# meiqua/pose_refine

Hardware: AMD Instinct MI355X
Metric: refined poses/sec (640x480, 20 ICP iters) (higher is better)
Workload: dtype f32; 1 GPU; obj_06.ply, 256-pose batch per GPU, 640x480 synthetic depth, projective association, 20 ICP iterations (21 passes), solve on device, 2 pose groups; poses_per_gpu=256, global_batch=256, parallelism=pose-shard x1, no data-path collective, no gather (1 rank)

## Files before the change

pose_refine_amd/csrc/icp_pass.hip:

```cpp
#include "pr_launch.h"
#include "icp_accumulate.h"
#include "icp_solve_device.h"

namespace prk {

template <class Scene, bool kNN, int kStack = 0, bool kRobust = false>
__global__ __launch_bounds__(256, PR_PASS_WAVES) void icp_pass_kernel(IcpBatch b, Scene scene)
{
    extern __shared__ __attribute__((aligned(16))) unsigned char lds_raw[];
    __shared__ float wsum[4][kAccStride];

    const uint32_t pose = blockIdx.y;
    const PoseMeta &pm = b.meta[pose];
    const int32_t st = pm.state;
    if (st == kSkip) return;
    const uint32_t n = pm.count;
    const uint32_t ppb = b.steps * kPointsPerStep;
    if ((uint64_t)blockIdx.x * ppb >= n) return;

    const int4 *lds_topo = nullptr;
    int *stk_node = nullptr; float *stk_lb = nullptr;
    if constexpr (kNN && kStack == 0) {
        int4 *dst = reinterpret_cast<int4 *>(lds_raw);
        for (uint32_t i = threadIdx.x; i < scene.lds_nodes; i += kBlockThreads) dst[i] = scene.topo[i];
// ... 44 lines not shown
    const float *p = partial + (size_t)pose * nblk * kAccStride + comp;
    for (uint32_t g0 = 0; g0 < used; g0 += 16) {
        float v[16];
#pragma unroll
        for (uint32_t k = 0; k < 16; ++k) v[k] = (g0 + k < used) ? p[(size_t)(g0 + k) * kAccStride] : 0.0f;
#pragma unroll
        for (uint32_t k = 0; k < 16; ++k) if (g0 + k < used) total += v[k];
    }
    return total;
}

constexpr uint32_t kLoopLanes = 1024, kLoopWaves = kLoopLanes / 64, kLoopHeader = 64;
static_assert(sizeof(DevIcpState) == 20 * sizeof(uint32_t), "the LDS header holds DevIcpState as 20 words");
size_t icp_loop_cu_lds_bytes(uint32_t nblk) { return ((size_t)nblk * 4 * kAccStride + kLoopHeader) * sizeof(float); }
uint32_t icp_loop_cu_lds_blocks(uint32_t nblk, uint32_t steps, int cap)
{
    const size_t fixed = icp_loop_cu_lds_bytes(nblk), block = (size_t)steps * kPointsPerStep * sizeof(pr_vec3);
    if (fixed > kLoopCuLdsBudget || block == 0) return 0;
    const size_t fit = (kLoopCuLdsTotal - fixed) / block;
    uint32_t r = (uint32_t)(fit < nblk ? fit : nblk);
    if (cap >= 0 && (uint32_t)cap < r) r = (uint32_t)cap;
    return r;
}

template <class Scene>
__global__ __launch_bounds__(kLoopLanes) PR_LOOP_CU_ATTR void icp_loop_cu_kernel(IcpBatch b, Scene scene)
{
    extern __shared__ __attribute__((aligned(16))) float loop_lds[];
    const uint32_t pose = blockIdx.x;
    const PoseMeta &pm = b.meta[pose];
    const int32_t st0 = pm.state;
    const uint32_t n = pm.count;
    if (st0 == kSkip || n == 0) return;
    const uint32_t ppb = b.steps * kPointsPerStep;
    const uint32_t items = ((n + ppb - 1) / ppb) * 4u;
    const uint32_t lane = threadIdx.x & 63u;
    const uint32_t wave = __builtin_amdgcn_readfirstlane(threadIdx.x >> 6);
    float *hdr = loop_lds + (size_t)b.nblk * 4 * kAccStride;
    uint32_t *hdw = reinterpret_cast<uint32_t *>(hdr);
    float *cl = reinterpret_cast<float *>(b.cloud + pm.start);
    float *lcl = hdr + kLoopHeader;
    const uint32_t lds_items = b.lds_blocks * 4u;
    bool xf = (st0 == kRunWithTransform) && !b.pre_transformed;
    float M[12];
#pragma unroll
    for (int i = 0; i < 12; ++i) M[i] = xf ? pm.xform[i] : 0.0f;
    if (wave == 0 && lane < 20) hdw[16 + lane] = reinterpret_cast<const uint32_t *>(b.st + pose)[lane];

    const uint32_t last_it = (uint32_t)b.crit.max_iteration;
    uint32_t it = 0;
    for (;; ++it) {
        const bool score_only = it == last_it;
        for (uint32_t item = wave; item < items; item += kLoopWaves) {
            const uint32_t vb = item >> 2, tib = ((item & 3u) << 6) | lane;
            float acc[29];
            float *row = loop_lds + (size_t)item * kAccStride;
            const bool in_lds = item < lds_items;
            if (score_only) {
                if (!in_lds) vb_accumulate_at<Scene, false, 0, true>(tib, acc, cl, cl, n, vb * ppb, b.steps, xf, M, scene, nullptr, nullptr, nullptr, nullptr, xf);
                else if (it == 0) vb_accumulate_at<Scene, false, 0, true, false, true>(tib, acc, cl, lcl, n, vb * ppb, b.steps, xf, M, scene, nullptr, nullptr, nullptr, nullptr, xf);
                else vb_accumulate_at<Scene, false, 0, true>(tib, acc, lcl, lcl, n, vb * ppb, b.steps, xf, M, scene, nullptr, nullptr, nullptr, nullptr, xf);
                wave_reduce<true>(acc, lane, row);
            } else {
                if (!in_lds) vb_accumulate_at<Scene, false, 0>(tib, acc, cl, cl, n, vb * ppb, b.steps, xf, M, scene, nullptr, nullptr, nullptr, nullptr, xf);
                else if (it == 0) vb_accumulate_at<Scene, false, 0, false, false, true>(tib, acc, cl, lcl, n, vb * ppb, b.steps, xf, M, scene, nullptr, nullptr, nullptr, nullptr, xf);
                else vb_accumulate_at<Scene, false, 0>(tib, acc, lcl, lcl, n, vb * ppb, b.steps, xf, M, scene, nullptr, nullptr, nullptr, nullptr, xf);
                wave_reduce(acc, lane, row);
            }
        }
        __syncthreads();
        if (wave == 0) {
            float total = 0.0f;
            if (lane < 29) {
                const float *r = loop_lds + lane;
                for (uint32_t i = 0; i < items; i += 4u, r += 4 * kAccStride)
                    total += ((r[0] + r[kAccStride]) + r[2 * kAccStride]) + r[3 * kAccStride];
            }
            DevIcpState s;
#pragma unroll
            for (int i = 0; i < 16; ++i) s.T[i] = hdr[16 + i];
            s.fitness = hdr[32]; s.rmse = hdr[33]; s.done = (int32_t)hdw[34]; s.passes = (int32_t)hdw[35];
            float E[16];
            const bool finished = pose_iteration_wave(total, n, s, b.crit, it, E);
            if (lane == 0) {
#pragma unroll
                for (int i = 0; i < 16; ++i) hdr[16 + i] = s.T[i];
                hdr[32] = s.fitness; hdr[33] = s.rmse; hdw[35] = (uint32_t)s.passes;
                if (!finished) {
#pragma unroll
                    for (int i = 0; i < 12; ++i) hdr[i] = E[i];
                }
                hdw[12] = (finished || it >= last_it) ? 1u : 0u;
            }
        }
        __syncthreads();
        if (__builtin_amdgcn_readfirstlane(hdw[12]) != 0u) break;
#pragma unroll
        for (int i = 0; i < 12; ++i) M[i] = __int_as_float(__builtin_amdgcn_readfirstlane(__float_as_int(hdr[i])));
        xf = true;
    }
    if (threadIdx.x == 0) {
        DevIcpState s;
#pragma unroll
        for (int i = 0; i < 16; ++i) s.T[i] = hdr[16 + i];
        s.fitness = hdr[32]; s.rmse = hdr[33]; s.done = 1; s.passes = (int32_t)hdw[35];
        b.st[pose] = s;
        PoseMeta *wm = const_cast<PoseMeta *>(b.meta) + pose;
        if (it > 0) {
#pragma unroll
            for (int i = 0; i < 12; ++i) wm->xform[i] = hdr[i];
        }
        wm->state = kSkip;
    }
}
hipError_t launch_icp_loop_cu_proj_packed(const IcpBatch &b, const SceneProjPacked &sc, uint32_t n_poses, hipStream_t s, uint32_t *lds_blocks_used)
{
    if (lds_blocks_used) *lds_blocks_used = 0;
    if (n_poses == 0 || b.nblk == 0) return hipSuccess;
    size_t lds = icp_loop_cu_lds_bytes(b.nblk);
    if (lds > kLoopCuLdsBudget || b.robust_kind != PR_ROBUST_NONE) return hipErrorInvalidValue;
    IcpBatch bb = b;
    const uint32_t most = icp_loop_cu_lds_blocks(b.nblk, b.steps, -1);
    if (bb.lds_blocks > most) bb.lds_blocks = most;
    const size_t image = (size_t)bb.lds_blocks * b.steps * kPointsPerStep * sizeof(pr_vec3);
    const auto fn = icp_loop_cu_kernel<SceneProjPacked>;
    if (lds + image > kLoopCuLdsBudget && !lds_opt_in(reinterpret_cast<const void *>(fn), 0, (uint32_t)kLoopCuLdsTotal)) bb.lds_blocks = 0;
    if (bb.lds_blocks) lds += image;
    if (lds_blocks_used) *lds_blocks_used = bb.lds_blocks;
    hipLaunchKernelGGL(HIP_KERNEL_NAME(icp_loop_cu_kernel<SceneProjPacked>), dim3(n_poses), dim3(kLoopLanes), lds, s, bb, sc);
    return hipGetLastError();
}

__global__ __launch_bounds__(64) void icp_finalize_kernel(const float *__restrict__ partial, const PoseMeta *__restrict__ meta,
                                                          uint32_t nblk, uint32_t ppb, float *__restrict__ sums)
{
    const uint32_t pose = blockIdx.x;
    if (meta[pose].state == kSkip) return;
    const uint32_t n = meta[pose].count;
    const uint32_t used = (n + ppb - 1) / ppb;
    if (threadIdx.x < kAccStride)
        sums[(size_t)pose * kAccStride + threadIdx.x] = (threadIdx.x < 29) ? sum_partials(partial, pose, nblk, used, threadIdx.x) : 0.0f;
}

__global__ __launch_bounds__(64) void icp_finalize_solve_kernel(const float *__restrict__ partial, PoseMeta *__restrict__ meta,
                                                                uint32_t nblk, uint32_t ppb, DevIcpState *__restrict__ st,
                                                                pr_criteria crit, uint32_t iter)
{
    const uint32_t pose = blockIdx.x;
    if (meta[pose].state == kSkip) return;
    const uint32_t n = meta[pose].count;
    const uint32_t used = (n + ppb - 1) / ppb;
    DevIcpState s = st[pose];
    float total = 0.0f;
// ... 163 lines not shown
```

pose_refine_amd/csrc/pr_context.cpp:

```cpp
#include "pr_runtime.h"

namespace prh {
thread_local std::string g_err;
void set_error(const char *fmt, ...)
{
    char buf[512];
    va_list ap; va_start(ap, fmt); vsnprintf(buf, sizeof buf, fmt, ap); va_end(ap);
    g_err = buf;
}
}

namespace prr {

static std::mutex &g_reg_mu_trace() { static std::mutex m; return m; }

namespace {
struct TraceRec { uint64_t ns; const char *tag; uint32_t tid; };
constexpr size_t kTraceCap = 1u << 18;
TraceRec *g_trace = nullptr;
std::atomic<uint64_t> g_trace_n{ 0 };
std::atomic<int> g_trace_state{ 0 };
std::string g_trace_path;
void trace_dump()
{
// ... 10 lines not shown
    if (st == 1) return;
    if (st == 0) {
        std::lock_guard<std::mutex> lk(g_reg_mu_trace());
        st = g_trace_state.load();
        if (st == 0) {
            const char *p = std::getenv("PR_TRACE");
            if (p && *p) { g_trace_path = p; g_trace = new TraceRec[kTraceCap]; std::atexit(trace_dump); st = 2; } else st = 1;
            g_trace_state.store(st, std::memory_order_release);
        }
        if (st == 1) return;
    }
    timespec ts; clock_gettime(CLOCK_MONOTONIC, &ts);
    static thread_local uint32_t tid = (uint32_t)std::hash<std::thread::id>()(std::this_thread::get_id());
    const uint64_t i = g_trace_n.fetch_add(1);
    if (i < kTraceCap) g_trace[i] = TraceRec{ (uint64_t)ts.tv_sec * 1000000000ull + (uint64_t)ts.tv_nsec, tag, tid };
}

WriteLog g_writes;
std::atomic<uint64_t> g_flag_overtook{ 0 };
std::atomic<uint64_t> g_tight_batches{ 0 };
std::atomic<uint64_t> g_band_batches{ 0 };
std::atomic<uint64_t> g_resident_batches{ 0 };
std::atomic<uint32_t> g_loop_lds_blocks{ 0 };
std::atomic<uint32_t> g_nn_lds_nodes{ 0 }, g_nn_stack_depth{ 0 };
std::atomic<uint64_t> g_nn_pass_launches{ 0 };
Options opt;
std::mutex g_reg_mu;
std::vector<Ctx *> g_shared;
int g_default_device = -1;
thread_local Ctx *g = nullptr;
thread_local PrivateCtx tl_private;
std::mutex g_private_mu;
std::vector<Ctx *> g_private;

void ctx_teardown(Ctx *c)
{
    if (!c->ready) return;
    (void)hipSetDevice(c->device);
    hipStreamSynchronize(c->stream);
    for (Slot &sl : c->slots) slot_release(sl);
    for (DevBuf *b : { &c->aabb, &c->aabb_keys, &c->bbox, &c->poses, &c->depth, &c->row_count, &c->row_off, &c->counts, &c->cloud, &c->meta, &c->partial,
                       &c->sums, &c->packed.rec, &c->nn_prev, &c->dstate, &c->dresults, &c->arrive, &c->conv16, &c->conv8, &c->kd_scratch, &c->kd_tmp, &c->nn_full, &c->gather_tmp, &c->nn_counters, &c->scores, &c->multi, &c->ov_bits, &c->ov_box, &c->ov_mat, &c->cov_state, &c->cov_claimed, &c->mesh_sorted, &c->mesh_verts, &c->contours, &c->normals, &c->cmp_keys, &c->cmp_box, &c->cmp_rec, &c->edge_bits, &c->edge_rows, &c->lvl_rows, &c->lvl_counts, &c->lvl_carry, &c->pd_mats, &c->pd_part, &c->pd_rec, &c->ppf_tmp, &c->ppf_out, &c->plane_tmp, &c->seg_tmp, &c->dfilt_tmp, &c->cloud_tmp, &c->vsd_rec, &c->solid_far, &c->solid_rec, &c->info_meta, &c->info_part }) b->release();
    for (NNDerived &d : c->nn_sets) d.release();
    for (PinBuf *b : { &c->h_sums, &c->h_meta, &c->h_counts, &c->h_results, &c->h_dstate, &c->h_poses, &c->h_flags, &c->h_scores, &c->h_multi, &c->h_ov, &c->h_cov, &c->h_contours, &c->h_normals, &c->h_lvl_carry, &c->h_cmp, &c->h_pd_mats, &c->h_pd_rec, &c->h_ppf, &c->h_plane, &c->h_seg, &c->h_dfilt, &c->h_vsd, &c->h_solid, &c->h_info_meta, &c->h_info_out }) b->release();
    c->packed = PackedCache();
    for (auto &gr : c->graphs) destroy_graph(gr);
// ... 189 lines not shown
    if (n == "solve") { if (value != PR_SOLVE_HOST && value != PR_SOLVE_DEVICE) { set_error("solve must be 0 or 1"); return PR_ERR_INVALID; } opt.solve_mode = value; }
    else if (n == "host_worker") opt.host_worker = value ? 1 : 0;
    else if (n == "start_overlap") opt.start_overlap = value;
    else if (n == "points_per_block") { if (value < 1024 || value % 1024) { set_error("points_per_block must be a multiple of 1024"); return PR_ERR_INVALID; } opt.steps = value / 1024; }
    else if (n == "profile") { if (value < 0 || value > 3) { set_error("profile must be 0, 1 (every launch, synchronous calls), 2 (every launch of one call in sample_period) or 3 (every launch, asynchronous batches stay asynchronous)"); return PR_ERR_INVALID; } opt.profile = value; }
    else if (n == "sample_period") opt.sample_period = std::max(1, value);
    else if (n == "scene_cache") opt.scene_cache = value ? 1 : 0;
    else if (n == "nn_lds_nodes") opt.nn_lds_nodes = std::max(0, value);
    else if (n == "nn_lds_records") opt.nn_lds_records = std::max(0, value);
    else if (n == "nn_compact") opt.nn_compact = value ? 1 : 0;
    else if (n == "nn_wide") opt.nn_wide = value ? 1 : 0;
    else if (n == "blocking_wait") opt.blocking_wait = value ? 1 : 0;
    else if (n == "nn_seed") opt.nn_seed = value ? 1 : 0;
    else if (n == "nn_stack") opt.nn_stack = value ? 1 : 0;
    else if (n == "nn_split") opt.nn_split = value ? 1 : 0;
    else if (n == "nn_run") opt.nn_run = std::min(8, std::max(1, value));
    else if (n == "nn_grid") opt.nn_grid = value ? 1 : 0;
    else if (n == "nn_count") opt.nn_count = value ? 1 : 0;
    else if (n == "host_poll") opt.host_poll = value ? 1 : 0;
    else if (n == "graph") opt.use_graph = value ? 1 : 0;
    else if (n == "fused_solve") opt.fused_solve = value ? 1 : 0;
    else if (n == "resident_loop") opt.resident_loop = value ? 1 : 0;
    else if (n == "loop_lds_blocks") opt.loop_lds_blocks = std::max(-1, value);
    else if (n == "sub_batch") opt.sub_batch = std::min(32768, std::max(32, value));
    else if (n == "overlap_pass") opt.overlap_pass = std::max(-1, value);
    else if (n == "pose_groups") opt.pose_groups = std::min(4, std::max(0, value));
    else if (n == "eager_streams") opt.eager_streams = value ? 1 : 0;
    else if (n == "mesh_order") opt.mesh_order = value ? 1 : 0;
    else if (n == "tight_box") opt.tight_box = value ? 1 : 0;
    else if (n == "box_bands") opt.box_bands = value ? 1 : 0;
    else if (n == "ppf_walk") opt.ppf_walk = value ? 1 : 0;
    else if (n == "raster_mode") { if (value < 0 || value > 1) { set_error("raster_mode must be 0 or 1"); return PR_ERR_INVALID; } opt.raster_mode = value; }
    else { set_error("unknown option %s", name); return PR_ERR_INVALID; }
    return PR_OK;
}

int pr_get_option(const char *name, int *value)
{
    std::lock_guard<std::mutex> lk(g_reg_mu);
    if (!name || !value) { set_error("pr_get_option: null argument"); return PR_ERR_INVALID; }
    const std::string n(name);
    if (n == "solve") *value = opt.solve_mode;
    else if (n == "host_worker") *value = opt.host_worker;
    else if (n == "start_overlap") *value = opt.start_overlap;
    else if (n == "points_per_block") *value = opt.steps * 1024;
    else if (n == "profile") *value = opt.profile;
// ... 7 lines not shown
    else if (n == "nn_seed") *value = opt.nn_seed;
    else if (n == "nn_stack") *value = opt.nn_stack;
    else if (n == "nn_split") *value = opt.nn_split;
    else if (n == "nn_run") *value = opt.nn_run;
    else if (n == "nn_grid") *value = opt.nn_grid;
    else if (n == "nn_count") *value = opt.nn_count;
    else if (n == "host_poll") *value = opt.host_poll;
    else if (n == "stat_flag_overtook") *value = (int)std::min<uint64_t>(g_flag_overtook.load(), 0x7fffffffull);
    else if (n == "stat_tight_batches") *value = (int)std::min<uint64_t>(g_tight_batches.load(), 0x7fffffffull);
    else if (n == "box_pack") *value = (int)prk::kBoxPack;
    else if (n == "pose_dist_chunk") *value = (int)prk::kPoseDistChunk;
    else if (n == "raster_mode") *value = opt.raster_mode;
    else if (n == "mesh_order") *value = opt.mesh_order;
    else if (n == "tight_box") *value = opt.tight_box;
    else if (n == "box_bands") *value = opt.box_bands;
    else if (n == "ppf_walk") *value = opt.ppf_walk;
    else if (n == "stat_band_batches") *value = (int)std::min<uint64_t>(g_band_batches.load(), 0x7fffffffull);
    else if (n == "eager_streams") *value = opt.eager_streams;
    else if (n == "graph") *value = opt.use_graph;
    else if (n == "fused_solve") *value = opt.fused_solve;
    else if (n == "resident_loop") *value = opt.resident_loop;
    else if (n == "loop_lds_blocks") *value = opt.loop_lds_blocks;
    else if (n == "stat_loop_lds_blocks") *value = (int)g_loop_lds_blocks.load();
    else if (n == "stat_nn_lds_nodes") *value = (int)g_nn_lds_nodes.load();
    else if (n == "stat_nn_stack_depth") *value = (int)g_nn_stack_depth.load();
    else if (n == "stat_nn_pass_launches") *value = (int)(g_nn_pass_launches.load() & 0x7fffffffull);
    else if (n == "stat_resident_batches") *value = (int)std::min<uint64_t>(g_resident_batches.load(), 0x7fffffffull);
    else if (n == "sub_batch") *value = opt.sub_batch;
    else if (n == "overlap_pass") *value = opt.overlap_pass;
    else if (n == "pose_groups") *value = opt.pose_groups;
    else { set_error("unknown option %s", name); return PR_ERR_INVALID; }
    return PR_OK;
}

int pr_profile_reset(void)
{
    PR_TRY(bind_default());
    std::lock_guard<std::mutex> lk(g->mu);
    g->icp_ms = g->render_ms = g->cloud_ms = 0; g->icp_launches = g->icp_points = g->icp_bytes = 0; g->sample_clock = 0;
    g->gather_ms = 0; g->gather_n = 0; g->gather_ev_used = 0;
    g->icp_launch_us.clear();
    for (double &v : g->nn_part_ms) v = 0;
    g->nn_part_n = 0;
    return PR_OK;
}

// ... 43 lines not shown
```

pose_refine_amd/csrc/pr_internal.h:

```cpp
#pragma once

#include <hip/hip_runtime_api.h>
#include <hip/hip_vector_types.h>
#include <stddef.h>
#include <stdint.h>
#include <vector>

#include "pose_refine.h"
#include "pr_tuning.h"

namespace prk {

constexpr uint32_t kBlockThreads   = 256;
constexpr uint32_t kPointsPerLane  = 4;
constexpr uint32_t kPointsPerStep  = kBlockThreads * kPointsPerLane;
constexpr uint32_t kAccStride      = 32;
constexpr uint32_t kCloudAlign     = 32;
constexpr uint32_t kBoxPack        = 32;
constexpr uint32_t kQCountStride   = 4;
constexpr uint32_t kNNWordsPerPoint = 6;

enum : int32_t { kSkip = 0, kRun = 1, kRunWithTransform = 2 };

struct alignas(64) PoseMeta {
// ... 26 lines not shown
    float          *nn_slack;
    uint2          *nn_queue;
    uint32_t       *nn_qcount;
    uint2          *nn_queue2;
    uint32_t        pre_transformed;
    pr_criteria     crit;
    uint32_t        robust_kind;
    float           robust_c, robust_inv_c;
    uint32_t        lds_blocks;
};
struct RobustArgs { uint32_t kind; float c, inv_c; float *corr; };

struct SceneProjAoS {
    uint32_t width, height;
    float max_dist_diff, fx, fy, cx, cy;
    float tlx, tly;
    const pr_vec3 *pcd, *normal;
};
struct SceneProjPacked {
    uint32_t width, height;
    float max_dist_diff, fx, fy, cx, cy;
    float tlx, tly;
    const float4 *rec;
    const float *colf, *rowf;
};
struct SceneNNDev {
    float max_dist_diff;
    const int4   *topo;
    const float4 *bmin, *bmax;
    const float4 *pts;
    const pr_vec3 *pcd, *normal;
    uint32_t n_nodes;
    uint32_t lds_nodes;
    const float4 *rec;
    uint32_t stack_depth;
    const uint4 *rec32;
    float qmin[3], qscale[3];
    const uint2 *desc;
    const float4 *grid;
    uint32_t gw, gh;
    float gfx, gfy, gcx, gcy;
    const float4 *pyr4, *pyr16, *pyr64;
    const uint4 *wide;
    uint32_t n_wide;
    float wmin[3], wscale;
    unsigned long long *counters;
// ... 139 lines not shown
hipError_t launch_stage_words(const void *src_host_mapped, void *dst, size_t bytes, hipStream_t s);
hipError_t launch_stage_words64(const void *src_host_mapped, void *dst, size_t bytes, hipStream_t s);
hipError_t launch_copy_words32(const void *src, void *dst, uint32_t n_words, hipStream_t s);
hipError_t launch_d2c_pack_starts(const uint32_t *counts, uint32_t n, PoseMeta *meta, hipStream_t s);
hipError_t launch_emit_box(const int32_t *depth, uint32_t n_poses, uint32_t width, uint32_t height, const int4 *bbox, float fx, float fy,
                           float cx, float cy, const uint32_t *row_count, const uint32_t *row_off, pr_vec3 *cloud, const PoseMeta *meta,
                           hipStream_t s, const uint32_t *box_off = nullptr, bool bands = false);

struct PyramidStrides { uint32_t n; uint32_t s[PR_PYRAMID_MAX_LEVELS]; };
struct alignas(64) PyramidCarry { float T[12]; uint32_t start; uint32_t pad[3]; };
static_assert(sizeof(PyramidCarry) == 64, "PyramidCarry must stay one 64-byte record");
hipError_t launch_pyramid_counts(const int32_t *depth, const int4 *bbox, const uint32_t *box_off, uint32_t n_poses, uint32_t width, uint32_t height,
                                 const PyramidStrides &lv, uint32_t *row_count, uint32_t *row_off, uint32_t *counts, hipStream_t s);
hipError_t launch_pyramid_emit(const int32_t *depth, uint32_t n_poses, uint32_t width, uint32_t height, const int4 *bbox, const uint32_t *box_off,
                               float fx, float fy, float cx, float cy, uint32_t stride, const uint32_t *row_count, const uint32_t *row_off,
                               const PyramidCarry *carry, bool apply, pr_vec3 *cloud, hipStream_t s);

hipError_t launch_icp_pass_proj_aos(const IcpBatch &b, const SceneProjAoS &sc, uint32_t n_poses, hipStream_t s);
hipError_t launch_icp_pass_proj_packed(const IcpBatch &b, const SceneProjPacked &sc, uint32_t n_poses, hipStream_t s);
constexpr size_t kLoopCuLdsBudget = 64u << 10;
size_t icp_loop_cu_lds_bytes(uint32_t nblk);
constexpr size_t kLoopCuLdsTotal = 160u << 10;
uint32_t icp_loop_cu_lds_blocks(uint32_t nblk, uint32_t steps, int cap);
hipError_t launch_icp_loop_cu_proj_packed(const IcpBatch &b, const SceneProjPacked &sc, uint32_t n_poses, hipStream_t s, uint32_t *lds_blocks_used = nullptr);
constexpr uint32_t kPassStaticLds = 4 * kAccStride * (uint32_t)sizeof(float);
constexpr uint32_t kNNLdsNodesMax = 8192;
constexpr uint32_t kNNLdsNodesPlain = ((64u << 10) - kPassStaticLds) / 16u;
struct NNPassRan { uint32_t lds_nodes, stack_depth; };
hipError_t launch_icp_pass_nn(const IcpBatch &b, const SceneNNDev &sc, uint32_t n_poses, hipStream_t s, NNPassRan *ran = nullptr);
hipError_t launch_nn_search(const IcpBatch &b, const SceneNNDev &sc, uint32_t n_poses, uint32_t max_points, uint32_t run, hipStream_t s, hipEvent_t *marks = nullptr);
hipError_t launch_icp_pass_nn_winners(const IcpBatch &b, const SceneNNWinners &sc, uint32_t n_poses, hipStream_t s);
hipError_t launch_icp_pass_grid(const IcpBatch &b, const SceneGridDev &sc, uint32_t n_poses, hipStream_t s);
hipError_t launch_grid_build(const SceneNNDev &tree, float reach, const SceneGridDev &grid, uint32_t *cell_point, hipStream_t s);
hipError_t launch_grid_records(const pr_vec3 *pcd, const pr_vec3 *normal, uint32_t n, float4 *rec, hipStream_t s);
hipError_t launch_contrib29_grid(pr_vec3 *cloud, uint32_t n, const float *update12, const SceneGridDev &sc, float *out, hipStream_t s);
hipError_t launch_contrib29_proj_aos(pr_vec3 *cloud, uint32_t n, const float *update12, const SceneProjAoS &sc, float *out, hipStream_t s);
hipError_t launch_contrib29_proj_packed(pr_vec3 *cloud, uint32_t n, const float *update12, const SceneProjPacked &sc, float *out, hipStream_t s);
hipError_t launch_contrib29_nn(pr_vec3 *cloud, uint32_t n, const float *update12, const SceneNNDev &sc, float *out, hipStream_t s);
hipError_t launch_robust_terms_proj_aos(pr_vec3 *cloud, uint32_t n, const float *update12, const SceneProjAoS &sc, const RobustArgs &ra, float *out, hipStream_t s);
hipError_t launch_robust_terms_proj_packed(pr_vec3 *cloud, uint32_t n, const float *update12, const SceneProjPacked &sc, const RobustArgs &ra, float *out, hipStream_t s);
hipError_t launch_robust_terms_nn(pr_vec3 *cloud, uint32_t n, const float *update12, const SceneNNDev &sc, const RobustArgs &ra, float *out, hipStream_t s);
hipError_t launch_robust_terms_grid(pr_vec3 *cloud, uint32_t n, const float *update12, const SceneGridDev &sc, const RobustArgs &ra, float *out, hipStream_t s);
hipError_t launch_pose_iteration_debug(const float *sums, const uint32_t *n_points, uint32_t n, pr_criteria crit, uint32_t iter, pr_result *state,
                                       float *update, uint32_t *finished, hipStream_t s);
size_t nn_grid_cells(uint32_t gw, uint32_t gh);
hipError_t launch_build_nn_grid(const pr_vec3 *pcd, uint32_t n_points, uint32_t gw, uint32_t gh, float fx, float fy, float cx, float cy,
                                int32_t *cell_idx, float4 *grid, uint32_t *usable, hipStream_t s);
// ... 84 lines not shown
```

pose_refine_amd/csrc/pr_refine.cpp:

```cpp
#include "pr_runtime.h"
#include "pose_box.h"

namespace prr {

int stage_poses(const pr_mat4 *poses_host, size_t n)
{
    PR_TRY(g->poses.ensure(sizeof(pr_mat4) * n));
    PR_TRY(g->h_poses.ensure(sizeof(pr_mat4) * n));
    std::memcpy(g->h_poses.p, poses_host, sizeof(pr_mat4) * n);
    HIP_TRY(prk::launch_stage_words(g->h_poses.dev, g->poses.p, sizeof(pr_mat4) * n, g->stream));
    return PR_OK;
}

uint32_t depth_chunk(size_t img, uint32_t P)
{
    return (uint32_t)std::max<size_t>(1, std::min<size_t>(P, ((size_t)4 << 30) / (img * sizeof(int32_t))));
}

std::pair<size_t, size_t> image_extent(pr_roi roi, size_t W, size_t H)
{
    if (roi.width > 0 && roi.height > 0) return { (size_t)roi.width, (size_t)roi.height };
    return { W, H };
}

// ... 910 lines not shown
    const prk::BoxRows rows{ sl.row_count.as<uint32_t>(), sl.row_off.as<uint32_t>(), sl.counts.as<uint32_t>() + q0, meta, dstate, arrive };
    HIP_TRY(prk::launch_render_boxes(mesh, d_poses + q0, nq, d_box + q0, target, rows, st, false, q0 == 0 ? &chk : nullptr));
    if (timed) { sl.spans.end(te, kSpanRender, q0, nq, false, st); te = sl.spans.begin(st); }
    HIP_TRY(prk::launch_emit_box(sl.depth.as<int32_t>(), nq, W, H, d_box + q0, K[0], K[4], K[2], K[5], sl.row_count.as<uint32_t>(),
                                 sl.row_off.as<uint32_t>(), sl.cloud.as<pr_vec3>(), meta, st, d_off + q0, bands));
    if (timed) sl.spans.end(te, kSpanCloud, q0, nq, false, st);
    if (timed && q0 == 0)
        for (Slot &o : g->slots) if (&o != &sl && o.pending && !o.delivered && o.done) HIP_TRY(hipStreamWaitEvent(st, o.done, 0));

    const uint32_t n_groups = pose_group_count(job.scene_kind, nq, timed);
    if (nn_prev) HIP_TRY(prk::launch_fill_i32(reinterpret_cast<int32_t *>(nn_prev + nl.qcount), (size_t)prk::kQCountStride * nq, 0, st));
    prk::IcpBatch b{};
    b.cloud = sl.cloud.as<pr_vec3>(); b.partial = sl.partial.as<float>(); b.nblk = pl.nblk; b.grid_x = pl.grid_x; b.steps = pl.steps;
    if (nn_prev) nn_carve(b, nn_prev, nl);
    const uint32_t last_pass = (uint32_t)job.crit.max_iteration;
    if (opt.resident_loop && opt.fused_solve && !timed && job.scene_kind == PR_SCENE_PROJ && sc.kind == PR_SCENE_PROJ && sc.packed
        && prk::icp_loop_cu_lds_bytes(pl.nblk) <= prk::kLoopCuLdsBudget) {
        b.meta = meta; b.st = dstate; b.crit = job.crit; b.fused = 1;
        const bool release = q0 + pl.sub >= P;
#if PR_RESIDENT_RELEASE_AHEAD
        if (release) { HIP_TRY(hipEventRecord(sl.progress, st)); sl.progress_valid = true; }
#endif
        b.lds_blocks = prk::icp_loop_cu_lds_blocks(pl.nblk, pl.steps, opt.loop_lds_blocks);
        uint32_t lds_blocks_used = 0;
        HIP_TRY(prk::launch_icp_loop_cu_proj_packed(b, sc.pk, nq, st, &lds_blocks_used));
        g_loop_lds_blocks.store(lds_blocks_used);
#if !PR_RESIDENT_RELEASE_AHEAD
        if (release) { HIP_TRY(hipEventRecord(sl.progress, st)); sl.progress_valid = true; }
#endif
        g_resident_batches.fetch_add(1);
        return PR_OK;
    }
    auto pass = [&](const prk::IcpBatch &bb, uint32_t p0, uint32_t np, hipStream_t gs) -> int {
        if (!timed) { HIP_TRY(launch_pass(bb, sc, np, gs)); return PR_OK; }
        const size_t e0 = sl.spans.begin(st);
        size_t mi[3] = { 0, 0, 0 }; hipEvent_t me[3] = { nullptr, nullptr, nullptr };
        const bool marks = sc.kind == PR_SCENE_NN && sc.nn_split && bb.nn_prev && np <= 32768u && sl.spans.reserve_marks(mi, me);
        HIP_TRY(launch_pass(bb, sc, np, gs, marks ? me : nullptr));
        sl.spans.end(e0, kSpanIcp, q0 + p0, np, bb.iter == 0 || bb.iter == last_pass, st, marks ? mi : nullptr);
        return PR_OK;
    };
    const uint32_t release_pass = release_pass_for(job.mesh.n_tris, nq, g->cloud_hint, job.crit, job.scene_kind, timed, pipeline_start, opt.start_overlap, opt.overlap_pass);
    auto after = [&](uint32_t it, bool &) -> int {
        if (q0 + pl.sub >= P && it == release_pass) { HIP_TRY(hipEventRecord(sl.progress, st)); sl.progress_valid = true; }
        return PR_OK;
    };
    const Lanes lanes{ sl.stream, sl.side, sl.fork, sl.join };
    return device_solve_loop(lanes, n_groups, b, nq, job.crit, opt.fused_solve != 0, meta, dstate, arrive, pass, after);
}
// ... 594 lines not shown
        if (rc == PR_OK) rc = make_job("pr_refine_submit", tris_dev, n_tris, width, height, proj, K, scene_kind, scene, crit, roi, results_dev, job);
        if (rc == PR_OK) rc = refine_submit(g->slots[slot], job, poses_host, n_poses, results_host, cloud_sizes_host);
    }
    trace_mark("pr_refine_submit: exit");
    return rc;
}

int pr_refine_submit(int slot, const pr_triangle *tris_dev, size_t n_tris, const pr_mat4 *poses_host, uint32_t n_poses, uint32_t width, uint32_t height,
                     const pr_mat4 *proj, const float K[9], int scene_kind, const void *scene, pr_criteria crit,
                     pr_result *results_host, pr_result *results_dev, uint32_t *cloud_sizes_host)
{
    return pr_refine_submit_roi(slot, tris_dev, n_tris, poses_host, n_poses, width, height, proj, K, scene_kind, scene, crit, pr_roi{ 0, 0, 0, 0 }, results_host, results_dev, cloud_sizes_host);
}

int pr_refine_wait(int slot)
{
    trace_mark("pr_refine_wait: enter");
    int rc;
    { PR_ENTER(); rc = refine_wait(slot); }
    trace_mark("pr_refine_wait: exit");
    return rc;
}

}
```

pose_refine_amd/csrc/pr_runtime.h:

```cpp
#pragma once
#include <hip/hip_runtime_api.h>
#include <rccl/rccl.h>
#include <dlfcn.h>

#include <algorithm>
#include <atomic>
#include <cfloat>
#include <cmath>
#include <cstdarg>
#include <cstdio>
#include <cstdlib>
#include <cstring>
#include <condition_variable>
#include <memory>
#include <mutex>
#include <thread>
#include <string>
#include <vector>

#include "pr_internal.h"
#include "pr_tuning.h"
#include "pose_box.h"
#include "contour_fit.h"

// ... 66 lines not shown
        if (bytes == 0) {
            void *base = nullptr; size_t size = 0;
            if (hipMemGetAddressRange(reinterpret_cast<hipDeviceptr_t *>(&base), &size, const_cast<void *>(p)) == hipSuccess && base) { lo = reinterpret_cast<uintptr_t>(base); hi = lo + size; }
            else { (void)hipGetLastError(); lo = 0; hi = ~(uintptr_t)0; }
        }
        std::lock_guard<std::mutex> lk(mu);
        ++gen;
        ring[gen % kRing] = W{ lo, hi };
    }
    uint64_t now() { std::lock_guard<std::mutex> lk(mu); return gen; }
    bool written_since(uint64_t since, const void *p, size_t bytes)
    {
        const uintptr_t lo = reinterpret_cast<uintptr_t>(p), hi = lo + bytes;
        std::lock_guard<std::mutex> lk(mu);
        if (gen - since >= kRing) return true;
        for (uint64_t k = since + 1; k <= gen; ++k) { const W &w = ring[k % kRing]; if (w.lo < hi && lo < w.hi) return true; }
        return false;
    }
};
extern WriteLog g_writes;
extern std::atomic<uint64_t> g_tight_batches;
extern std::atomic<uint64_t> g_band_batches;
extern std::atomic<uint64_t> g_resident_batches;
extern std::atomic<uint32_t> g_loop_lds_blocks;
extern std::atomic<uint32_t> g_nn_lds_nodes, g_nn_stack_depth;
extern std::atomic<uint64_t> g_nn_pass_launches;
extern std::atomic<uint64_t> g_flag_overtook;

constexpr int kSlots = PR_SLOTS;
struct Options {
    int pose_groups = 0;
    int solve_mode = PR_SOLVE_HOST;
    int host_worker = 1;
    int steps = 3;
    int profile = 0;
    int sample_period = 32;
    int nn_lds_nodes = 1024;
    int nn_lds_records = 0;
    int nn_seed = 1;
    int nn_compact = 1;
    int blocking_wait = 0;
    int nn_wide = 1;
    int nn_stack = 1;
    int nn_split = 1;
    int nn_run = 8;
    int nn_grid = 1;
    int host_poll = 1;
    int nn_count = 0;
    int start_overlap = -1;
    int overlap_pass = -1;
    int sub_batch = 512;
    int fused_solve = 1;
    int resident_loop = 1;
    int loop_lds_blocks = -1;
    int use_graph = 1;
    int eager_streams = 1;
    int raster_mode = 0;
    int mesh_order = 1;
    int tight_box = 1;
    int box_bands = 1;
    int ppf_walk = 1;
    int scene_cache = 1;
};
extern Options opt;
inline uint32_t pose_groups_for(int scene_kind) { (void)scene_kind; return opt.pose_groups > 0 ? (uint32_t)opt.pose_groups : 2u; }

struct ProjTail { uint32_t exact; prk::FpWords fp; uint32_t pad[3]; };
static_assert(sizeof(ProjTail) == 32, "ProjTail: the 32 bytes behind the tables");
struct PackedLayout { size_t colf, rowf, tail, bytes; };
inline PackedLayout packed_layout(size_t w, size_t h)
{
    PackedLayout l{};
    l.colf = w * h * sizeof(float4); l.rowf = l.colf + w * sizeof(float);
    l.tail = l.colf + (((w + h) * sizeof(float) + 15) & ~(size_t)15); l.bytes = l.tail + sizeof(ProjTail);
    return l;
}
// ... 820 lines not shown
```

pose_refine_amd/csrc/pr_tuning.h:

```cpp
#pragma once

#ifndef PR_SLOTS
#define PR_SLOTS 2
#endif

#ifndef PR_RESIDENT_RELEASE_AHEAD
#define PR_RESIDENT_RELEASE_AHEAD 1
#endif

#ifndef PR_LOOP_CU_WAVES
#define PR_LOOP_CU_WAVES 0
#endif
#if PR_LOOP_CU_WAVES
#define PR_LOOP_CU_ATTR __attribute__((amdgpu_waves_per_eu(PR_LOOP_CU_WAVES, PR_LOOP_CU_WAVES)))
#else
#define PR_LOOP_CU_ATTR
#endif

#ifndef PR_PASS_WAVES
#define PR_PASS_WAVES 1
#endif
#ifndef PR_GRID_PASS_WAVES
#define PR_GRID_PASS_WAVES 1
#endif
#ifndef PR_PASS_PREFETCH
#define PR_PASS_PREFETCH 0
#endif
#ifndef PR_PASS_LATE_STORE
#define PR_PASS_LATE_STORE 1
#endif
#ifndef PR_HOST_ROW_TAG
#define PR_HOST_ROW_TAG 1
#endif
#ifndef PR_PASS_TAIL_PRIO
// ... 92 lines not shown
```

pose_refine_amd/csrc/proj_query.h:

```cpp
#pragma once
#include "pr_device.h"

namespace prk {

__device__ __forceinline__ float div_normal_range(float a, float b)
{
    float r = __builtin_amdgcn_rcpf(b);
    const float e0 = __builtin_fmaf(-b, r, 1.0f);
    r = __builtin_fmaf(e0, r, r);
    float q = a * r;
    const float e1 = __builtin_fmaf(-b, q, a);
    q = __builtin_fmaf(e1, r, q);
    const float e2 = __builtin_fmaf(-b, q, a);
    return __builtin_fmaf(e2, r, q);
}

__device__ __forceinline__ bool proj_pixel(float sx, float sy, float sz, float fx, float fy, float cx, float cy, float tlx, float tly,
                                           uint32_t width, uint32_t height, uint32_t &idx, int &px, int &py)
{
    constexpr float kScale = 0x1p64f;
    const float zs = sz * kScale;
    float r = __builtin_amdgcn_rcpf(zs);
    const float e0 = __builtin_fmaf(-zs, r, 1.0f);
    r = __builtin_fmaf(e0, r, r);
// ... 59 lines not shown
    const float adiff = (diff > 0) ? diff : -diff;
    if (!in_img || dz <= 0 || adiff > s.max_dist_diff) return false;
    c.dx = g.a0; c.dy = g.a1; c.dz = dz; c.nx = g.b0; c.ny = g.b1; c.nz = g.b2;
    return true;
}
__device__ __forceinline__ bool gather_issue(const SceneProjPacked &s, float sx, float sy, float sz, bool live, Gathered &g)
{
    uint32_t idx = 0u; int px = 0, py = 0;
    const bool in_img = live && proj_pixel(sx, sy, sz, s.fx, s.fy, s.cx, s.cy, s.tlx, s.tly, s.width, s.height, idx, px, py);
    const float4 r = ld_off<float4>(s.rec, idx * 16u);
    g.a0 = r.x; g.a1 = r.y; g.a2 = r.z; g.a3 = r.w;
    g.b0 = ld_off<float>(s.colf, (uint32_t)px * 4u); g.b1 = ld_off<float>(s.rowf, (uint32_t)py * 4u); g.b2 = 0.0f;
    return in_img;
}
__device__ __forceinline__ bool gather_finish(const SceneProjPacked &s, bool in_img, float sz, const Gathered &g, Corr &c)
{
    const float dz = g.a3;
    const float diff = sz - dz;
    const float adiff = (diff > 0) ? diff : -diff;
    if (!in_img || dz <= 0 || adiff > s.max_dist_diff) return false;
    c.dx = g.b0 * dz; c.dy = g.b1 * dz; c.dz = dz; c.nx = g.a0; c.ny = g.a1; c.nz = g.a2;
    return true;
}
__device__ __forceinline__ bool gather_issue(const SceneNNDev &, float, float, float, bool, Gathered &) { return false; }
__device__ __forceinline__ bool gather_finish(const SceneNNDev &, bool, float, const Gathered &, Corr &) { return false; }
__device__ __forceinline__ bool gather_issue(const SceneNNWinners &, float, float, float, bool, Gathered &) { return false; }
__device__ __forceinline__ bool gather_finish(const SceneNNWinners &, bool, float, const Gathered &, Corr &) { return false; }

}
```

Before: 347,000 poses/s.

## Add half-width resident loop kernel and stage intrinsic tables in LDS

Result: faster. 379,200 poses/s, median of 6 (+9.3%).

```diff
diff --git a/pose_refine_amd/csrc/icp_pass.hip b/pose_refine_amd/csrc/icp_pass.hip
--- a/pose_refine_amd/csrc/icp_pass.hip
+++ b/pose_refine_amd/csrc/icp_pass.hip
@@ -90,10 +90,39 @@
     if (cap >= 0 && (uint32_t)cap < r) r = (uint32_t)cap;
     return r;
 }
-
-template <class Scene>
-__global__ __launch_bounds__(kLoopLanes) PR_LOOP_CU_ATTR void icp_loop_cu_kernel(IcpBatch b, Scene scene)
-{
+__host__ __device__ constexpr uint32_t loop_table_words(uint32_t width, uint32_t height) { return (width + height + 3u) & ~3u; }
+uint32_t icp_loop_cu_layout(uint32_t nblk, uint32_t steps, int cap, uint32_t width, uint32_t height, uint32_t waves, uint32_t *fixed_bytes)
+{
+    const size_t limit = waves >= kLoopWaves ? kLoopCuLdsTotal : kLoopCuLdsTotal / 2;
+    const size_t rows = icp_loop_cu_lds_bytes(nblk), block = (size_t)steps * kPointsPerStep * sizeof(pr_vec3);
+    size_t tables = (size_t)loop_table_words(width, height) * sizeof(float);
+    if (fixed_bytes) *fixed_bytes = (uint32_t)rows;
+    if (rows > kLoopCuLdsBudget || rows > limit || block == 0) return 0;
+    auto blocks_behind = [&](size_t fixed) {
+        const size_t fit = (limit - fixed) / block;
+        uint32_t r = (uint32_t)(fit < nblk ? fit : nblk);
+        if (cap >= 0 && (uint32_t)cap < r) r = (uint32_t)cap;
+        return r;
+    };
+    if (rows + tables > limit) tables = 0;
+    if (fixed_bytes) *fixed_bytes = (uint32_t)(rows + tables);
+    return blocks_behind(rows + tables);
+}
+
+template <bool kTables> struct LoopScene;
+template <> struct LoopScene<false> {
+    using type = SceneProjPacked;
+    static __device__ __forceinline__ const type &make(const SceneProjPacked &sc, const float *) { return sc; }
+};
+template <> struct LoopScene<true> {
+    using type = SceneProjPackedLds;
+    static __device__ __forceinline__ type make(const SceneProjPacked &sc, const float *tab) { return type{ sc, tab, tab + sc.width }; }
+};
+
+template <uint32_t kWaves, bool kTables>
+__device__ __forceinline__ void icp_loop_cu_body(const IcpBatch &b, const SceneProjPacked &scene_arg)
+{
+    using Scene = typename LoopScene<kTables>::type;
     extern __shared__ __attribute__((aligned(16))) float loop_lds[];
     const uint32_t pose = blockIdx.x;
     const PoseMeta &pm = b.meta[pose];
@@ -107,19 +136,33 @@
     float *hdr = loop_lds + (size_t)b.nblk * 4 * kAccStride;
     uint32_t *hdw = reinterpret_cast<uint32_t *>(hdr);
     float *cl = reinterpret_cast<float *>(b.cloud + pm.start);
-    float *lcl = hdr + kLoopHeader;
+    float *tab = hdr + kLoopHeader;
+    float *lcl = tab + (kTables ? loop_table_words(scene_arg.width, scene_arg.height) : 0u);
     const uint32_t lds_items = b.lds_blocks * 4u;
     bool xf = (st0 == kRunWithTransform) && !b.pre_transformed;
     float M[12];
 #pragma unroll
     for (int i = 0; i < 12; ++i) M[i] = xf ? pm.xform[i] : 0.0f;
     if (wave == 0 && lane < 20) hdw[16 + lane] = reinterpret_cast<const uint32_t *>(b.st + pose)[lane];
+    if constexpr (kTables) {
+        const uint32_t w = scene_arg.width, wh = w + scene_arg.height;
+        for (uint32_t i = threadIdx.x; i < wh; i += kWaves * 64u) tab[i] = i < w ? scene_arg.colf[i] : scene_arg.rowf[i - w];
+        __syncthreads();
+    }
+    const Scene scene = LoopScene<kTables>::make(scene_arg, tab);
+#if PR_LOOP_CU_PROBE
+    uint64_t probe_serial = 0, probe_total = 0;
+#endif
 
     const uint32_t last_it = (uint32_t)b.crit.max_iteration;
     uint32_t it = 0;
     for (;; ++it) {
         const bool score_only = it == last_it;
-        for (uint32_t item = wave; item < items; item += kLoopWaves) {
+#if PR_LOOP_CU_PROBE
+        const uint64_t probe_t0 = wall_clock64();
+        uint64_t probe_t1 = 0;
+#endif
+        for (uint32_t item = wave; item < items; item += kWaves) {
             const uint32_t vb = item >> 2, tib = ((item & 3u) << 6) | lane;
             float acc[29];
             float *row = loop_lds + (size_t)item * kAccStride;
@@ -137,6 +180,9 @@
             }
         }
         __syncthreads();
+#if PR_LOOP_CU_PROBE
+        probe_t1 = wall_clock64();
+#endif
         if (wave == 0) {
             float total = 0.0f;
             if (lane < 29) {
@@ -161,7 +207,13 @@
                 hdw[12] = (finished || it >= last_it) ? 1u : 0u;
             }
         }
+#if PR_LOOP_CU_PROBE
+        probe_serial += wall_clock64() - probe_t1;
+#endif
         __syncthreads();
+#if PR_LOOP_CU_PROBE
+        probe_total += wall_clock64() - probe_t0;
+#endif
         if (__builtin_amdgcn_readfirstlane(hdw[12]) != 0u) break;
 #pragma unroll
         for (int i = 0; i < 12; ++i) M[i] = __int_as_float(__builtin_amdgcn_readfirstlane(__float_as_int(hdr[i])));
@@ -179,24 +231,44 @@
             for (int i = 0; i < 12; ++i) wm->xform[i] = hdr[i];
         }
         wm->state = kSkip;
-    }
-}
-hipError_t launch_icp_loop_cu_proj_packed(const IcpBatch &b, const SceneProjPacked &sc, uint32_t n_poses, hipStream_t s, uint32_t *lds_blocks_used)
-{
-    if (lds_blocks_used) *lds_blocks_used = 0;
+#if PR_LOOP_CU_PROBE
+        float *pr = b.partial + (size_t)pose * 4;
+        pr[0] = (float)probe_serial; pr[1] = (float)probe_total; pr[2] = (float)(it + 1u); pr[3] = (float)items;
+#endif
+    }
+}
+template <bool kTables>
+__global__ __launch_bounds__(kLoopLanes) PR_LOOP_CU_ATTR void icp_loop_cu_kernel(IcpBatch b, SceneProjPacked scene) { icp_loop_cu_body<kLoopWaves, kTables>(b, scene); }
+template <bool kTables>
+__global__ __launch_bounds__(kLoopLanes / 2) __attribute__((amdgpu_waves_per_eu(4, 4))) void icp_loop_cu8_kernel(IcpBatch b, SceneProjPacked scene) { icp_loop_cu_body<kLoopWaves / 2, kTables>(b, scene); }
+hipError_t launch_icp_loop_cu_proj_packed(const IcpBatch &b, const SceneProjPacked &sc, uint32_t n_poses, hipStream_t s, LoopCuForm form, LoopCuUsed *used)
+{
+    if (used) *used = LoopCuUsed{ 0, 0, 0 };
     if (n_poses == 0 || b.nblk == 0) return hipSuccess;
-    size_t lds = icp_loop_cu_lds_bytes(b.nblk);
-    if (lds > kLoopCuLdsBudget || b.robust_kind != PR_ROBUST_NONE) return hipErrorInvalidValue;
+    const size_t rows = icp_loop_cu_lds_bytes(b.nblk);
+    if (rows > kLoopCuLdsBudget || b.robust_kind != PR_ROBUST_NONE) return hipErrorInvalidValue;
+    const uint32_t waves = form.waves == kLoopWaves / 2 ? kLoopWaves / 2 : kLoopWaves;
+    const bool want_tables = form.tables < 0 ? waves != kLoopWaves : form.tables != 0;
     IcpBatch bb = b;
-    const uint32_t most = icp_loop_cu_lds_blocks(b.nblk, b.steps, -1);
-    if (bb.lds_blocks > most) bb.lds_blocks = most;
-    const size_t image = (size_t)bb.lds_blocks * b.steps * kPointsPerStep * sizeof(pr_vec3);
-    const auto fn = icp_loop_cu_kernel<SceneProjPacked>;
-    if (lds + image > kLoopCuLdsBudget && !lds_opt_in(reinterpret_cast<const void *>(fn), 0, (uint32_t)kLoopCuLdsTotal)) bb.lds_blocks = 0;
-    if (bb.lds_blocks) lds += image;
-    if (lds_blocks_used) *lds_blocks_used = bb.lds_blocks;
-    hipLaunchKernelGGL(HIP_KERNEL_NAME(icp_loop_cu_kernel<SceneProjPacked>), dim3(n_poses), dim3(kLoopLanes), lds, s, bb, sc);
-    return hipGetLastError();
+    uint32_t fixed = 0;
+    bb.lds_blocks = icp_loop_cu_layout(b.nblk, b.steps, (int)(b.lds_blocks < b.nblk ? b.lds_blocks : b.nblk), want_tables ? sc.width : 0u, want_tables ? sc.height : 0u, waves, &fixed);
+    const size_t block = (size_t)b.steps * kPointsPerStep * sizeof(pr_vec3);
+    bool tables = fixed > rows;
+    const void *fn = waves == kLoopWaves ? (tables ? reinterpret_cast<const void *>(icp_loop_cu_kernel<true>) : reinterpret_cast<const void *>(icp_loop_cu_kernel<false>))
+                                         : (tables ? reinterpret_cast<const void *>(icp_loop_cu8_kernel<true>) : reinterpret_cast<const void *>(icp_loop_cu8_kernel<false>));
+    const int slot = waves == kLoopWaves ? (tables ? 3 : 0) : (tables ? 5 : 4);
+    const size_t limit = waves == kLoopWaves ? kLoopCuLdsTotal : kLoopCuLdsTotal / 2;
+    if (fixed + bb.lds_blocks * block > kLoopCuLdsBudget && !lds_opt_in(fn, slot, (uint32_t)limit)) {
+        bb.lds_blocks = 0;
+        if (fixed > kLoopCuLdsBudget) {
+            tables = false; fixed = (uint32_t)rows;
+            fn = waves == kLoopWaves ? reinterpret_cast<const void *>(icp_loop_cu_kernel<false>) : reinterpret_cast<const void *>(icp_loop_cu8_kernel<false>);
+        }
+    }
+    const size_t lds = fixed + bb.lds_blocks * block;
+    if (used) *used = LoopCuUsed{ bb.lds_blocks, waves, tables ? fixed - (uint32_t)rows : 0u };
+    void *args[] = { &bb, const_cast<SceneProjPacked *>(&sc) };
+    return hipLaunchKernel(fn, dim3(n_poses), dim3(waves * 64u), args, lds, s);
 }
 
 __global__ __launch_bounds__(64) void icp_finalize_kernel(const float *__restrict__ partial, const PoseMeta *__restrict__ meta,
diff --git a/pose_refine_amd/csrc/pr_context.cpp b/pose_refine_amd/csrc/pr_context.cpp
--- a/pose_refine_amd/csrc/pr_context.cpp
+++ b/pose_refine_amd/csrc/pr_context.cpp
@@ -56,6 +56,8 @@
 std::atomic<uint64_t> g_band_batches{ 0 };
 std::atomic<uint64_t> g_resident_batches{ 0 };
 std::atomic<uint32_t> g_loop_lds_blocks{ 0 };
+std::atomic<uint32_t> g_loop_waves{ 0 };
+std::atomic<uint32_t> g_loop_lds_tables{ 0 };
 std::atomic<uint32_t> g_nn_lds_nodes{ 0 }, g_nn_stack_depth{ 0 };
 std::atomic<uint64_t> g_nn_pass_launches{ 0 };
 Options opt;
@@ -291,6 +293,8 @@
     else if (n == "fused_solve") opt.fused_solve = value ? 1 : 0;
     else if (n == "resident_loop") opt.resident_loop = value ? 1 : 0;
     else if (n == "loop_lds_blocks") opt.loop_lds_blocks = std::max(-1, value);
+    else if (n == "loop_lds_tables") opt.loop_lds_tables = std::min(1, std::max(-1, value));
+    else if (n == "loop_waves") { if (value != 0 && value != 8 && value != 16) { set_error("loop_waves must be 0, 8 or 16"); return PR_ERR_INVALID; } opt.loop_waves = value; }
     else if (n == "sub_batch") opt.sub_batch = std::min(32768, std::max(32, value));
     else if (n == "overlap_pass") opt.overlap_pass = std::max(-1, value);
     else if (n == "pose_groups") opt.pose_groups = std::min(4, std::max(0, value));
@@ -344,6 +348,10 @@
     else if (n == "resident_loop") *value = opt.resident_loop;
     else if (n == "loop_lds_blocks") *value = opt.loop_lds_blocks;
     else if (n == "stat_loop_lds_blocks") *value = (int)g_loop_lds_blocks.load();
+    else if (n == "loop_lds_tables") *value = opt.loop_lds_tables;
+    else if (n == "stat_loop_lds_tables") *value = (int)g_loop_lds_tables.load();
+    else if (n == "loop_waves") *value = opt.loop_waves;
+    else if (n == "stat_loop_waves") *value = (int)g_loop_waves.load();
     else if (n == "stat_nn_lds_nodes") *value = (int)g_nn_lds_nodes.load();
     else if (n == "stat_nn_stack_depth") *value = (int)g_nn_stack_depth.load();
     else if (n == "stat_nn_pass_launches") *value = (int)(g_nn_pass_launches.load() & 0x7fffffffull);
diff --git a/pose_refine_amd/csrc/pr_internal.h b/pose_refine_amd/csrc/pr_internal.h
--- a/pose_refine_amd/csrc/pr_internal.h
+++ b/pose_refine_amd/csrc/pr_internal.h
@@ -72,6 +72,10 @@
     float max_dist_diff, fx, fy, cx, cy;
     float tlx, tly;
     const float4 *rec;
+    const float *colf, *rowf;
+};
+struct SceneProjPackedLds {
+    SceneProjPacked pk;
     const float *colf, *rowf;
 };
 struct SceneNNDev {
@@ -257,7 +261,10 @@
 size_t icp_loop_cu_lds_bytes(uint32_t nblk);
 constexpr size_t kLoopCuLdsTotal = 160u << 10;
 uint32_t icp_loop_cu_lds_blocks(uint32_t nblk, uint32_t steps, int cap);
-hipError_t launch_icp_loop_cu_proj_packed(const IcpBatch &b, const SceneProjPacked &sc, uint32_t n_poses, hipStream_t s, uint32_t *lds_blocks_used = nullptr);
+uint32_t icp_loop_cu_layout(uint32_t nblk, uint32_t steps, int cap, uint32_t width, uint32_t height, uint32_t waves, uint32_t *fixed_bytes);
+struct LoopCuForm { uint32_t waves; int tables; };
+struct LoopCuUsed { uint32_t lds_blocks, waves, table_bytes; };
+hipError_t launch_icp_loop_cu_proj_packed(const IcpBatch &b, const SceneProjPacked &sc, uint32_t n_poses, hipStream_t s, LoopCuForm form, LoopCuUsed *used = nullptr);
 constexpr uint32_t kPassStaticLds = 4 * kAccStride * (uint32_t)sizeof(float);
 constexpr uint32_t kNNLdsNodesMax = 8192;
 constexpr uint32_t kNNLdsNodesPlain = ((64u << 10) - kPassStaticLds) / 16u;
diff --git a/pose_refine_amd/csrc/pr_refine.cpp b/pose_refine_amd/csrc/pr_refine.cpp
--- a/pose_refine_amd/csrc/pr_refine.cpp
+++ b/pose_refine_amd/csrc/pr_refine.cpp
@@ -956,9 +956,12 @@
         if (release) { HIP_TRY(hipEventRecord(sl.progress, st)); sl.progress_valid = true; }
 #endif
         b.lds_blocks = prk::icp_loop_cu_lds_blocks(pl.nblk, pl.steps, opt.loop_lds_blocks);
-        uint32_t lds_blocks_used = 0;
-        HIP_TRY(prk::launch_icp_loop_cu_proj_packed(b, sc.pk, nq, st, &lds_blocks_used));
-        g_loop_lds_blocks.store(lds_blocks_used);
+        const uint32_t waves = opt.loop_waves ? (uint32_t)opt.loop_waves : (nq >= (uint32_t)g->n_cus ? PR_LOOP_CU_FULL_CHIP_WAVES : 16u);
+        prk::LoopCuUsed used{};
+        HIP_TRY(prk::launch_icp_loop_cu_proj_packed(b, sc.pk, nq, st, prk::LoopCuForm{ waves, opt.loop_lds_tables }, &used));
+        g_loop_lds_blocks.store(used.lds_blocks);
+        g_loop_waves.store(used.waves);
+        g_loop_lds_tables.store(used.table_bytes);
 #if !PR_RESIDENT_RELEASE_AHEAD
         if (release) { HIP_TRY(hipEventRecord(sl.progress, st)); sl.progress_valid = true; }
 #endif
@@ -1599,4 +1602,15 @@
     return rc;
 }
 
-}
+#if PR_LOOP_CU_PROBE
+int pr_loop_probe_read(int slot, float *out, uint32_t n_poses)
+{
+    PR_ENTER();
+    if (slot < 0 || slot >= kSlots || !out) return PR_ERR_INVALID;
+    HIP_TRY(hipDeviceSynchronize());
+    HIP_TRY(hipMemcpy(out, g->slots[slot].partial.as<float>(), sizeof(float) * 4 * n_poses, hipMemcpyDeviceToHost));
+    return PR_OK;
+}
+#endif
+
+}
diff --git a/pose_refine_amd/csrc/pr_runtime.h b/pose_refine_amd/csrc/pr_runtime.h
--- a/pose_refine_amd/csrc/pr_runtime.h
+++ b/pose_refine_amd/csrc/pr_runtime.h
@@ -112,6 +112,8 @@
 extern std::atomic<uint64_t> g_tight_batches;
 extern std::atomic<uint64_t> g_band_batches;
 extern std::atomic<uint64_t> g_resident_batches;
+extern std::atomic<uint32_t> g_loop_waves;
+extern std::atomic<uint32_t> g_loop_lds_tables;
 extern std::atomic<uint32_t> g_loop_lds_blocks;
 extern std::atomic<uint32_t> g_nn_lds_nodes, g_nn_stack_depth;
 extern std::atomic<uint64_t> g_nn_pass_launches;
@@ -142,6 +144,8 @@
     int sub_batch = 512;
     int fused_solve = 1;
     int resident_loop = 1;
+    int loop_lds_tables = -1;
+    int loop_waves = 0;
     int loop_lds_blocks = -1;
     int use_graph = 1;
     int eager_streams = 1;
diff --git a/pose_refine_amd/csrc/pr_tuning.h b/pose_refine_amd/csrc/pr_tuning.h
--- a/pose_refine_amd/csrc/pr_tuning.h
+++ b/pose_refine_amd/csrc/pr_tuning.h
@@ -10,6 +10,12 @@
 
 #ifndef PR_LOOP_CU_WAVES
 #define PR_LOOP_CU_WAVES 0
+#endif
+#ifndef PR_LOOP_CU_FULL_CHIP_WAVES
+#define PR_LOOP_CU_FULL_CHIP_WAVES 8u
+#endif
+#ifndef PR_LOOP_CU_PROBE
+#define PR_LOOP_CU_PROBE 0
 #endif
 #if PR_LOOP_CU_WAVES
 #define PR_LOOP_CU_ATTR __attribute__((amdgpu_waves_per_eu(PR_LOOP_CU_WAVES, PR_LOOP_CU_WAVES)))
diff --git a/pose_refine_amd/csrc/proj_query.h b/pose_refine_amd/csrc/proj_query.h
--- a/pose_refine_amd/csrc/proj_query.h
+++ b/pose_refine_amd/csrc/proj_query.h
@@ -105,6 +105,19 @@
     c.dx = g.b0 * dz; c.dy = g.b1 * dz; c.dz = dz; c.nx = g.a0; c.ny = g.a1; c.nz = g.a2;
     return true;
 }
+__device__ __forceinline__ bool gather_issue(const SceneProjPackedLds &s, float sx, float sy, float sz, bool live, Gathered &g)
+{
+    uint32_t idx = 0u; int px = 0, py = 0;
+    const bool in_img = live && proj_pixel(sx, sy, sz, s.pk.fx, s.pk.fy, s.pk.cx, s.pk.cy, s.pk.tlx, s.pk.tly, s.pk.width, s.pk.height, idx, px, py);
+    const float4 r = ld_off<float4>(s.pk.rec, idx * 16u);
+    g.a0 = r.x; g.a1 = r.y; g.a2 = r.z; g.a3 = r.w;
+    g.b0 = ld_off<float>(s.colf, (uint32_t)px * 4u); g.b1 = ld_off<float>(s.rowf, (uint32_t)py * 4u); g.b2 = 0.0f;
+    return in_img;
+}
+__device__ __forceinline__ bool gather_finish(const SceneProjPackedLds &s, bool in_img, float sz, const Gathered &g, Corr &c)
+{
+    return gather_finish(s.pk, in_img, sz, g, c);
+}
 __device__ __forceinline__ bool gather_issue(const SceneNNDev &, float, float, float, bool, Gathered &) { return false; }
 __device__ __forceinline__ bool gather_finish(const SceneNNDev &, bool, float, const Gathered &, Corr &) { return false; }
 __device__ __forceinline__ bool gather_issue(const SceneNNWinners &, float, float, float, bool, Gathered &) { return false; }
```
